# Bioconductor/SparseArray

Hardware: NVIDIA B200
Metric: nnz/s for SVT colSums+colMeans+rowSums+rowVars (na.rm=TRUE), 33538x1e6 int counts d=0.07 per GPU (higher is better)
Workload: dtype int32->f64

## Files before the change

### sparsearray_b200/csrc/svtgpu_colstats.cu

```cuda
#include "svtgpu_internal.h"
#include "svt_ptx.cuh"

#include <stdlib.h>
#include <string.h>

namespace {

enum ColClass { CC_COUNT = 0, CC_SUM, CC_MINMAX, CC_VAR, CC_ANYALL, CC_PROD };

__host__ __device__ inline int col_class_of(int opcode)
{
	switch (opcode) {
	    case SVTGPU_OP_ANYNA: case SVTGPU_OP_COUNTNAS: return CC_COUNT;
	    case SVTGPU_OP_SUM: case SVTGPU_OP_MEAN:       return CC_SUM;
	    case SVTGPU_OP_MIN: case SVTGPU_OP_MAX:        return CC_MINMAX;
	    case SVTGPU_OP_CENTERED_X2_SUM:
	    case SVTGPU_OP_VAR1: case SVTGPU_OP_SD1:       return CC_VAR;
	    case SVTGPU_OP_ANY: case SVTGPU_OP_ALL:        return CC_ANYALL;
	    case SVTGPU_OP_PROD:                           return CC_PROD;
	}
	return -1;
}

struct ColParams {
// ... 330 lines not shown
				}
			}
			for (; i < n; i++) {
				const int x = (int) p[i * 32];
				const bool na = x == SVT_NA_INT;
				const int x0 = na ? 0 : x;
				nna += na;
				s1 += x0;
				s2 += (unsigned int) (x0 * x0);
			}
			SvtColPartial sp;
			svt_col_partial_init(&sp);
			sp.nz = end - start;
			sp.n_na = svt_warp_sum((long long) nna);
			sp.sum = (double) svt_warp_sum((long long) s1);
			unsigned long long t2 = s2;
#pragma unroll
			for (int m = 16; m > 0; m >>= 1)
				t2 += __shfl_xor_sync(SVT_FULL_MASK, t2, m);
			if (lane == 0)
				store_result(P, seg, var_from_int_sums(P.opcode,
						P.narm, P.seg_len, &sp, t2));
			continue;
		}
		LaneAcc<CC, T> acc;
		acc.reset();
		lane_accumulate<CC, T>(acc, vals, start, end, lane);
		SvtColPartial part;
		acc.reduce_into(&part, end - start);
		double center = P.center;
		if (CC == CC_VAR && sizeof(T) == 4 && svt_isnan(center)) {
			int amax = acc.imax;
			unsigned long long s2 = acc.isum2;
#pragma unroll
			for (int m = 16; m > 0; m >>= 1) {
				const int o = __shfl_xor_sync(SVT_FULL_MASK,
							      amax, m);
				amax = o > amax ? o : amax;
				s2 += __shfl_xor_sync(SVT_FULL_MASK, s2, m);
			}
			if (amax < 65536) {
				if (lane == 0)
					store_result(P, seg, var_from_int_sums(
						P.opcode, P.narm, P.seg_len,
						&part, s2));
				continue;
			}
		}
		if (CC == CC_VAR) {
			const bool about_mean = svt_isnan(center);
			if (about_mean)
				center = svt_col_mean(P.is_double, P.narm,
						      P.seg_len, &part);
			bool one_pass = false;
			if (sizeof(T) == 8 && about_mean && P.var_onepass) {
				const double S2 = svt_warp_sum(acc.dsum2);
				const int64_t n_reg = part.nz - part.n_na - part.n_nan;
				const int64_t n = P.seg_len -
					(P.narm ? part.n_na + part.n_nan : 0);
				if (S2 >= 1e-200 && S2 <= 1e200 && n > 0 &&
				    4 * n_reg <= n && !svt_isnan(center)) {
					part.sum2 = S2 - 2.0 * center * part.sum +
						    (double) n_reg * center * center;
					one_pass = true;
				}
			}
			if (!one_pass) {
				double s2 = 0.0;
#pragma unroll 4
				for (int64_t e = start + lane; e < end; e += 32)
					add_sq(s2, vals[e], center);
				part.sum2 = svt_warp_sum(s2);
			}
		}
		if (lane == 0)
			store_result(P, seg, svt_col_finalize(P.opcode,
					P.is_double, P.narm, P.seg_len, center,
					&part));
	}
}

__device__ __forceinline__ void sum_i8_word(uint32_t w, int &s, int &na_bits)
{
	s = __dp4a((int) w, 0x01010101, s);
	na_bits += __popc(__vcmpeq4(w, 0x80808080u));
}

#define SUM_I8_BLOCKS_PER_SM 6
__global__ void __launch_bounds__(256, SUM_I8_BLOCKS_PER_SM)
colstats_sum_i8(ColParams P, const int8_t *__restrict__ v8)
{
	const int lane = threadIdx.x & 31;
	const int64_t warps = ((int64_t) gridDim.x * blockDim.x) >> 5;
	const int64_t gw = ((int64_t) blockIdx.x * blockDim.x + threadIdx.x) >> 5;
	int64_t nstart = 0, nend = 0;
	if (gw < P.nseg) {
		nstart = P.leaf_ptr[gw * P.group];
		nend = P.leaf_ptr[(gw + 1) * P.group];
	}
	for (int64_t seg = gw; seg < P.nseg; seg += warps) {
		const int64_t start = nstart, end = nend;
		if (seg + warps < P.nseg) {
			nstart = P.leaf_ptr[(seg + warps) * P.group];
			nend = P.leaf_ptr[(seg + warps + 1) * P.group];
		}
		long long sum = 0;
		int na_bits = 0;
		const int64_t a16 = (start + 15) & ~(int64_t) 15;
		const int64_t b16 = end & ~(int64_t) 15;
		int64_t lo = start, hi = end;
		if (a16 < b16) {
			const uint4 *q = (const uint4 *) (v8 + a16);
			const int nv = (int) ((b16 - a16) >> 4);
			for (int i = lane; i < nv; i += 128) {
				uint4 u[4];
#pragma unroll
				for (int k = 0; k < 4; k++)
					u[k] = i + 32 * k < nv ? __ldcs(q + i + 32 * k)
							       : make_uint4(0, 0, 0, 0);
				int s = 0;
#pragma unroll
				for (int k = 0; k < 4; k++) {
					sum_i8_word(u[k].x, s, na_bits);
					sum_i8_word(u[k].y, s, na_bits);
					sum_i8_word(u[k].z, s, na_bits);
					sum_i8_word(u[k].w, s, na_bits);
				}
				sum += s;
			}
			if (start + lane < a16) {
				const int x = v8[start + lane];
				sum += x;
				na_bits += x == SVT_COMPACT_NA_I8 ? 8 : 0;
			}
			lo = b16;
		}
		for (int64_t e = lo + lane; e < hi; e += 32) {
			const int x = v8[e];
			sum += x;
			na_bits += x == SVT_COMPACT_NA_I8 ? 8 : 0;
		}
		const long long n_na = svt_warp_sum((long long) na_bits) >> 3;
		sum = svt_warp_sum(sum) + 128 * n_na;
		if (lane == 0) {
			SvtColPartial part;
			svt_col_partial_init(&part);
			part.nz = end - start;
			part.n_na = n_na;
			part.sum = (double) sum;
			store_result(P, seg, svt_col_finalize(P.opcode, P.is_double,
					P.narm, P.seg_len, P.center, &part));
		}
	}
}


#define COL_NS 2

enum {
	IT_FIRST = 1,
	IT_PASS_END = 2,
	IT_PASS2 = 4,
	IT_LAST = 8,
	IT_SINGLE = 16,
	IT_STOP = 32
};

struct __align__(16) ItemMeta {
	int64_t seg;
	int64_t start, end;
	int64_t cbase;
	int32_t celems;
	int32_t flags;
};

template <int CC, typename T>
__device__ __forceinline__ void consume_pass1(LaneAcc<CC, T> &acc,
		const T *buf, int lo, int hi, int lane)
{
	constexpr int VN = Vec16<T>::N;
	const int lo_v = (lo + VN - 1) / VN * VN;
	const int hi_v = hi / VN * VN;
	if (lo_v >= hi_v) {
		for (int e = lo + lane; e < hi; e += 32)
			acc.add(buf[e]);
		return;
	}
	if (lo + lane < lo_v)
		acc.add(buf[lo + lane]);
	if (hi_v + lane < hi)
		acc.add(buf[hi_v + lane]);
	const Vec16<T> *vb = (const Vec16<T> *) buf;
#pragma unroll 2
	for (int v = lo_v / VN + lane; v < hi_v / VN; v += 32) {
		Vec16<T> x = vb[v];
#pragma unroll
		for (int i = 0; i < VN; i++)
			acc.add(x.get(i));
	}
}

template <typename T>
__device__ __forceinline__ void consume_pass2(double &s2, const T *buf,
		int lo, int hi, int lane, double c)
{
	constexpr int VN = Vec16<T>::N;
	const int lo_v = (lo + VN - 1) / VN * VN;
	const int hi_v = hi / VN * VN;
	if (lo_v >= hi_v) {
		for (int e = lo + lane; e < hi; e += 32)
			add_sq(s2, buf[e], c);
		return;
	}
	if (lo + lane < lo_v)
		add_sq(s2, buf[lo + lane], c);
	if (hi_v + lane < hi)
		add_sq(s2, buf[hi_v + lane], c);
	const Vec16<T> *vb = (const Vec16<T> *) buf;
#pragma unroll 2
	for (int v = lo_v / VN + lane; v < hi_v / VN; v += 32) {
		Vec16<T> x = vb[v];
#pragma unroll
		for (int i = 0; i < VN; i++)
			add_sq(s2, x.get(i), c);
	}
}

template <int CC, typename T>
__global__ void __launch_bounds__(512, 1)
colstats_tma(ColParams P, int pairs, int stage_bytes)
{
	extern __shared__ __align__(128) unsigned char smem[];
	unsigned char *data = smem;
	ItemMeta *metas = (ItemMeta *) (smem + (size_t) pairs * COL_NS *
							 stage_bytes);
	uint64_t *bars = (uint64_t *) (metas + pairs * COL_NS);

	const int warp = threadIdx.x >> 5;
	const int lane = threadIdx.x & 31;
	const int pair = warp >> 1;
	const bool is_producer = (warp & 1) == 0;

	if (threadIdx.x == 0) {
		for (int i = 0; i < 2 * pairs * COL_NS; i++)
			svt_mbar_init(svt_smem_u32(&bars[i]), 1);
		svt_mbar_init_fence();
	}
	__syncthreads();

	unsigned char *ring = data + (size_t) pair * COL_NS * stage_bytes;
	ItemMeta *meta = metas + pair * COL_NS;
	const uint32_t full0 = svt_smem_u32(&bars[pair * COL_NS]);
	const uint32_t empty0 = svt_smem_u32(&bars[(pairs + pair) * COL_NS]);
	const int64_t npairs_total = (int64_t) gridDim.x * pairs;
	const int64_t gp = (int64_t) blockIdx.x * pairs + pair;
	constexpr int SZ = (int) sizeof(T);

	if (is_producer) {
		if (lane != 0)
			return;
		const char *vals = (const char *) P.vals;
		const uint64_t policy = svt_policy_evict_first();
		uint32_t it = 0;
		int64_t seg = gp;
		int64_t nstart = 0, nend = 0;
		if (seg < P.nseg) {
			nstart = P.leaf_ptr[seg * P.group];
			nend = P.leaf_ptr[(seg + 1) * P.group];
		}
		while (seg < P.nseg) {
			const int64_t start = nstart, end = nend;
			const int64_t next = seg + npairs_total;
			if (next < P.nseg) {
				nstart = P.leaf_ptr[next * P.group];
				nend = P.leaf_ptr[(next + 1) * P.group];
			}
			const int64_t a0 = (start * SZ) & ~(int64_t) 15;
			const int64_t a1 = (end * SZ + 15) & ~(int64_t) 15;
			const int64_t nch = start == end ? 0
				: (a1 - a0 + stage_bytes - 1) / stage_bytes;
			const int npass = (CC == CC_VAR && nch > 1) ? 2 : 1;
			const int64_t nitems = nch == 0 ? 1 : nch * npass;
			int64_t k = 0;
			for (int pass = 0; pass < npass; pass++) {
			    for (int64_t ch = 0; ch < (nch == 0 ? 1 : nch);
				 ch++, k++) {
				const int st = it % COL_NS;
				svt_mbar_wait(empty0 + 8 * st,
					      ((it / COL_NS) & 1) ^ 1);
				const int64_t ca = a0 + ch * stage_bytes;
				int64_t cb = ca + stage_bytes;
				if (cb > a1) cb = a1;
				const uint32_t bytes = nch == 0 ? 0
						: (uint32_t) (cb - ca);
				ItemMeta md;
				md.seg = seg;
				md.start = start;
				md.end = end;
				md.cbase = ca / SZ;
				md.celems = (int32_t) (bytes / SZ);
				md.flags = (k == 0 ? IT_FIRST : 0) |
					(ch + 1 >= nch ? IT_PASS_END : 0) |
					(pass == 1 ? IT_PASS2 : 0) |
					(k + 1 == nitems ? IT_LAST : 0) |
					(nch <= 1 ? IT_SINGLE : 0);
				meta[st] = md;
// ... 58 lines not shown
				}
			}
		} else {
			consume_pass2<T>(s2, buf, lo, hi, lane, center);
		}
		if (md.flags & IT_LAST) {
			if (CC == CC_VAR)
				part.sum2 = svt_warp_sum(s2);
			if (lane == 0)
				store_result(P, md.seg, svt_col_finalize(
					P.opcode, P.is_double, P.narm,
					P.seg_len, center, &part));
		}
		__syncwarp();
		if (lane == 0)
			svt_mbar_arrive(empty0 + 8 * st);
	}
}

__global__ void __launch_bounds__(256)
colstats_lacunar(ColParams P)
{
	const int64_t stride = (int64_t) gridDim.x * blockDim.x;
	for (int64_t seg = (int64_t) blockIdx.x * blockDim.x + threadIdx.x;
	     seg < P.nseg; seg += stride) {
		const int64_t nz = P.leaf_ptr[(seg + 1) * P.group] -
				   P.leaf_ptr[seg * P.group];
		SvtColPartial part;
		svt_col_partial_ones(&part, nz, 0.0);
		double center = P.center;
		if (svt_col_op_needs_center(P.opcode)) {
			if (svt_isnan(center))
				center = svt_col_mean(P.is_double, P.narm,
						      P.seg_len, &part);
			svt_col_partial_ones(&part, nz, center);
		}
		store_result(P, seg, svt_col_finalize(P.opcode, P.is_double,
				P.narm, P.seg_len, center, &part));
	}
}

template <typename T>
int launch_typed(const ColParams &P, int cc, bool use_tma, int avg_seg_bytes,
		 cudaStream_t stream)
{
	const int sms = svtgpu_sm_count();
	if (!use_tma) {
		int64_t blocks = (P.nseg + 7) / 8;
		if (blocks > (int64_t) sms * 8) blocks = (int64_t) sms * 8;
		if (blocks < 1) blocks = 1;
#define DIRECT(CC) colstats_direct<CC, T><<<(unsigned) blocks, 256, 0, stream>>>(P)
		switch (cc) {
		    case CC_COUNT:  DIRECT(CC_COUNT); break;
		    case CC_SUM:    DIRECT(CC_SUM); break;
		    case CC_MINMAX: DIRECT(CC_MINMAX); break;
		    case CC_VAR:    DIRECT(CC_VAR); break;
		    case CC_ANYALL: DIRECT(CC_ANYALL); break;
		    case CC_PROD:   DIRECT(CC_PROD); break;
		}
#undef DIRECT
		SVT_CUDA(cudaGetLastError());
		svtgpu_count_launch(1);
		return SVTGPU_OK;
	}
	int stage_bytes = (avg_seg_bytes + avg_seg_bytes / 4 + 64 + 1023) /
			  1024 * 1024;
	const int stage_env = atoi(svtgpu_env("SVTGPU_COL_STAGE_KB", "0"));
	if (stage_env > 0) stage_bytes = stage_env * 1024;
	if (stage_bytes < 4096) stage_bytes = 4096;
	if (stage_bytes > 48 * 1024) stage_bytes = 48 * 1024;
	int pairs = (200 * 1024) / (COL_NS * stage_bytes);
	if (pairs > 8) pairs = 8;
	if (pairs < 1) pairs = 1;
	const int pairs_env = atoi(svtgpu_env("SVTGPU_COL_PAIRS", "0"));
	if (pairs_env > 0 && pairs_env <= 8) pairs = pairs_env;
	const size_t smem = (size_t) pairs * COL_NS * stage_bytes +
			    (size_t) pairs * COL_NS * sizeof(ItemMeta) +
			    (size_t) 2 * pairs * COL_NS * sizeof(uint64_t);
	int64_t blocks = (P.nseg + pairs - 1) / pairs;
	if (blocks > sms) blocks = sms;
	if (blocks < 1) blocks = 1;
#define TMA(CC) do { \
		SVT_CUDA(cudaFuncSetAttribute(colstats_tma<CC, T>, \
			cudaFuncAttributeMaxDynamicSharedMemorySize, (int) smem)); \
		colstats_tma<CC, T><<<(unsigned) blocks, pairs * 64, smem, stream>>>( \
			P, pairs, stage_bytes); \
	} while (0)
	switch (cc) {
	    case CC_COUNT:  TMA(CC_COUNT); break;
	    case CC_SUM:    TMA(CC_SUM); break;
	    case CC_MINMAX: TMA(CC_MINMAX); break;
	    case CC_VAR:    TMA(CC_VAR); break;
	    case CC_ANYALL: TMA(CC_ANYALL); break;
	    case CC_PROD:   TMA(CC_PROD); break;
	}
#undef TMA
	SVT_CUDA(cudaGetLastError());
	svtgpu_count_launch(1);
	return SVTGPU_OK;
}

}

int svtgpu_launch_colstats(svtgpu_matrix *m, int opcode, int narm,
			   double center, int64_t group, void *d_out,
			   int32_t *d_warn, cudaStream_t stream)
{
	SVT_ARG(svt_col_op_supported(opcode, m->val_type),
		"colStats: operation %d is not supported on type %d by the "
		"GPU path", opcode, m->val_type);
	SVT_ARG(group >= 1 && (m->nleaf % group) == 0,
		"colStats: 'group' must divide the number of leaves");
	ColParams P;
	P.vals = m->d_vals;
	P.leaf_ptr = m->d_leaf_ptr;
	P.nseg = m->nleaf / group;
	P.group = group;
	P.seg_len = m->nrow * group;
	P.opcode = opcode;
	P.narm = narm != 0;
	P.is_double = svt_is_double(m->val_type);
	P.center = center;
	P.out = d_out;
	P.warn = d_warn;
	P.var_small = 0;
	P.var_onepass = strcmp(svtgpu_env("SVTGPU_COLVAR_DOUBLE", "auto"),
			       "twopass") != 0;
	if (!P.is_double && svt_isnan(center)) {
		const int64_t B = svtgpu_value_bound(m);
		const int64_t per_lane = P.seg_len / 32 + 2;
		if (B >= 0 && B < 46340 &&
		    per_lane < (int64_t) 0x7FFFFFFF / (B * B + 1)) {
			P.var_small = 1;
			if (m->vmax_abs >= 0 && m->vmin >= 0 &&
			    strcmp(svtgpu_env("SVTGPU_COLVAR_NONNEG", "on"),
				   "on") == 0)
				P.var_small = 2;
		}
	}
	if (P.nseg == 0)
		return SVTGPU_OK;
	if (!(m->flags & SVTGPU_HAS_VALS)) {
		int64_t blocks = (P.nseg + 255) / 256;
		int64_t cap = (int64_t) svtgpu_sm_count() * 8;
		if (blocks > cap) blocks = cap;
		colstats_lacunar<<<(unsigned) blocks, 256, 0, stream>>>(P);
		SVT_CUDA(cudaGetLastError());
		svtgpu_count_launch(1);
		return SVTGPU_OK;
	}
	const int cc = col_class_of(opcode);
	if (cc == CC_SUM && !P.is_double) {
		SVT_CHECK(svt_ensure_compact(m, stream));
		if (m->d_vals8 != NULL) {
			int64_t blocks = (P.nseg + 7) / 8;
			const int64_t cap = (int64_t) svtgpu_sm_count() *
					    SUM_I8_BLOCKS_PER_SM;
			if (blocks > cap)
				blocks = cap;
			colstats_sum_i8<<<(unsigned) blocks, 256, 0, stream>>>(
				P, m->d_vals8);
			SVT_CUDA(cudaGetLastError());
			svtgpu_count_launch(1);
			return SVTGPU_OK;
		}
	}
	const char *impl = svtgpu_env("SVTGPU_COLSTATS_IMPL", "direct");
	bool use_tma = strcmp(impl, "tma") == 0 &&
		       (((uintptr_t) m->d_vals) & 15) == 0;
	int64_t avg = m->nnz / P.nseg * (int64_t) svt_val_size(m->val_type);
	if (avg > (1 << 30)) avg = 1 << 30;
	if (P.is_double)
		return launch_typed<double>(P, cc, use_tma, (int) avg, stream);
	return launch_typed<int32_t>(P, cc, use_tma, (int) avg, stream);
}

extern "C" int svtgpu_colstats_out_is_int(int opcode, int val_type)
{
	return svt_col_out_is_int(opcode, val_type);
}

extern "C" int svtgpu_colstats_dev(svtgpu_matrix *m, int opcode, int narm,
				   double center, int64_t group, void *d_out,
				   int32_t *d_warn, void *stream)
{
	SVT_CHECK(svtgpu_require_device());
	SVT_ARG(m != NULL && d_out != NULL, "svtgpu_colstats_dev: NULL argument");
	return svtgpu_launch_colstats(m, opcode, narm, center, group, d_out,
				      d_warn, (cudaStream_t) stream);
}

extern "C" int svtgpu_colstats(svtgpu_matrix *m, int opcode, int narm,
			       double center, int64_t group, void *out,
			       int *warn)
{
	SVT_CHECK(svtgpu_require_device());
	SVT_ARG(m != NULL && out != NULL, "svtgpu_colstats: NULL argument");
	SVT_ARG(group >= 1 && (m->nleaf % group) == 0,
		"colStats: 'group' must divide the number of leaves");
	const int64_t nseg = m->nleaf / group;
	const size_t esz = svt_col_out_is_int(opcode, m->val_type) ? 4 : 8;
	if (warn != NULL)
		*warn = 0;
	m->tm.kernel_ms = m->tm.d2h_ms = 0.0;
	m->tm.d2h_bytes = 0.0;
	m->tm.launches = 0;
	if (nseg == 0)
		return SVTGPU_OK;
	void *scratch = NULL;
	SVT_CHECK(svtgpu_scratch(m, esz * (size_t) nseg + 16, &scratch));
	int32_t *d_warn = (int32_t *) scratch;
	void *d_out = (char *) scratch + 16;
	cudaStream_t s = 0;
	SVT_CUDA(cudaMemsetAsync(d_warn, 0, 16, s));
	SvtTimer t;
	SVT_CHECK(svt_timer_begin(&t, s));
	int64_t l0 = svtgpu_launch_count();
	int rc = svtgpu_launch_colstats(m, opcode, narm, center, group, d_out,
					d_warn, s);
	int rc2 = svt_timer_end(&t, &m->tm.kernel_ms);
	if (rc != SVTGPU_OK)
		return rc;
	SVT_CHECK(rc2);
	m->tm.launches = (int) (svtgpu_launch_count() - l0);
	SVT_CHECK(svt_timer_begin(&t, s));
	int32_t h_warn = 0;
	SVT_CUDA(cudaMemcpyAsync(out, d_out, esz * (size_t) nseg,
				 cudaMemcpyDeviceToHost, s));
	SVT_CUDA(cudaMemcpyAsync(&h_warn, d_warn, sizeof(int32_t),
				 cudaMemcpyDeviceToHost, s));
	SVT_CHECK(svt_timer_end(&t, &m->tm.d2h_ms));
	m->tm.d2h_bytes = (double) (esz * (size_t) nseg);
	if (warn != NULL)
		*warn = h_warn != 0;
	return SVTGPU_OK;
}

namespace {

template <int CC, typename T>
__global__ void __launch_bounds__(256)
summarize_slices(const T *__restrict__ vals, int64_t nnz, int64_t slice,
		 double center, int pass2, SvtColPartial *__restrict__ parts)
{
	const int lane = threadIdx.x & 31;
	const int64_t gw = ((int64_t) blockIdx.x * blockDim.x + threadIdx.x) >> 5;
	const int64_t start = gw * slice;
	if (start >= nnz)
		return;
	const int64_t end = start + slice < nnz ? start + slice : nnz;
	SvtColPartial part;
	if (pass2) {
		double s2 = 0.0;
#pragma unroll 4
		for (int64_t e = start + lane; e < end; e += 32)
			add_sq(s2, vals[e], center);
		svt_col_partial_init(&part);
		part.sum2 = svt_warp_sum(s2);
	} else {
		LaneAcc<CC, T> acc;
		acc.reset();
		lane_accumulate<CC, T>(acc, vals, start, end, lane);
		acc.reduce_into(&part, end - start);
	}
	if (lane == 0)
		parts[gw] = part;
}

__device__ __forceinline__ void col_partial_merge(SvtColPartial *a,
						  const SvtColPartial *b)
{
	a->nz += b->nz;
	a->n_na += b->n_na;
	a->n_nan += b->n_nan;
	a->n_zero += b->n_zero;
	a->sum += b->sum;
	a->sum2 += b->sum2;
	a->prod *= b->prod;
	a->vmin = b->vmin < a->vmin ? b->vmin : a->vmin;
	a->vmax = b->vmax > a->vmax ? b->vmax : a->vmax;
}

__device__ __forceinline__ void col_partial_warp_merge(SvtColPartial *acc)
{
	acc->nz = svt_warp_sum((long long) acc->nz);
	acc->n_na = svt_warp_sum((long long) acc->n_na);
	acc->n_nan = svt_warp_sum((long long) acc->n_nan);
	acc->n_zero = svt_warp_sum((long long) acc->n_zero);
	acc->sum = svt_warp_sum(acc->sum);
	acc->sum2 = svt_warp_sum(acc->sum2);
	acc->prod = svt_warp_prod(acc->prod);
	acc->vmin = svt_warp_min(acc->vmin);
	acc->vmax = svt_warp_max(acc->vmax);
}

__global__ void __launch_bounds__(1024)
summarize_combine(const SvtColPartial *__restrict__ parts, int64_t n,
		  SvtColPartial *__restrict__ out)
{
	__shared__ SvtColPartial warp_part[32];
	const int lane = threadIdx.x & 31;
	const int warp = threadIdx.x >> 5;
	SvtColPartial acc;
	svt_col_partial_init(&acc);
	for (int64_t i = threadIdx.x; i < n; i += blockDim.x) {
		const SvtColPartial p = parts[i];
// ... 301 lines not shown
```

### sparsearray_b200/csrc/svtgpu_internal.h

```cpp
#ifndef SVTGPU_INTERNAL_H
#define SVTGPU_INTERNAL_H

#include <cuda_runtime.h>
#include <stdint.h>
#include <stdio.h>

#include "../../include/svtgpu.h"
#include "svt_semantics.h"

#define SVTGPU_NSTAGE 3
#define SVTGPU_NSPLIT 4

struct svtgpu_matrix {
	int64_t nrow, nleaf, nnz;
	int val_type;
	int flags;
	int owns;
	int device;

	int64_t *d_leaf_ptr;
	int32_t *d_offs;
	void *d_vals;

	cudaStream_t up_stream;
	int64_t stage_cap;
	int32_t *h_offs_stage[SVTGPU_NSTAGE];
	void *h_vals_stage[SVTGPU_NSTAGE];
	cudaEvent_t stage_done[SVTGPU_NSTAGE];
	int stage_busy[SVTGPU_NSTAGE];
	int stage_cur;
	cudaEvent_t up_begin, up_end;
	int up_begun;
	void *d_narrow[SVTGPU_NSTAGE];
	size_t narrow_bytes;

	void *d_scratch;
	size_t scratch_bytes;
	int32_t *d_split[SVTGPU_NSPLIT];
	int split_tile_rows[SVTGPU_NSPLIT];
	int split_ntiles[SVTGPU_NSPLIT];
	int split_next;
	int64_t *d_hist_tiles;
	int64_t hist_tile, hist_ntiles;
	int hist_max_leaves;
	int64_t vmax_abs;
	int64_t n_i8_commits, n_wide_commits;
	int64_t vmin;
	int64_t leaf_base;
	struct svtgpu_matrix *transposed;
	int transpose_failed;
	uint16_t *d_offs16;
	int8_t *d_vals8;
	int compact_state;
	int compact_uses;

	svtgpu_timings tm;
};

#define SVT_COMPACT_NA_I8 (-128)
#define SVT_COMPACT_PAD 64
#define SVT_COMPACT_NONE 0
#define SVT_COMPACT_BUILT 1
#define SVT_COMPACT_INELIGIBLE 2
#define SVT_COMPACT_MAX_ABS 127
#define SVT_COMPACT_MAX_NROW 65536

int svt_ensure_compact(svtgpu_matrix *m, cudaStream_t s);
void svt_drop_compact(svtgpu_matrix *m, cudaStream_t s);

int64_t svtgpu_value_bound(const svtgpu_matrix *m);

void svtgpu_set_error(const char *fmt, ...);
int svtgpu_cuda_fail(cudaError_t e, const char *what, const char *file,
		     int line);

#define SVT_CUDA(call) \
	do { \
		cudaError_t e__ = (call); \
		if (e__ != cudaSuccess) \
			return svtgpu_cuda_fail(e__, #call, __FILE__, __LINE__); \
	} while (0)

#define SVT_CHECK(call) \
	do { \
		int rc__ = (call); \
		if (rc__ != SVTGPU_OK) \
			return rc__; \
	} while (0)

#define SVT_ARG(cond, ...) \
	do { \
		if (!(cond)) { \
			svtgpu_set_error(__VA_ARGS__); \
			return SVTGPU_ERR_ARG; \
		} \
	} while (0)

cudaError_t svt_malloc_async(void **out, size_t bytes, cudaStream_t s);
cudaError_t svt_free_async(void *p, cudaStream_t s);

int svtgpu_require_device(void);
void svtgpu_count_launch(int n);
int svtgpu_scratch(svtgpu_matrix *m, size_t bytes, void **ptr);
int svtgpu_sm_count(void);
const char *svtgpu_env(const char *name, const char *dflt);

static inline int svt_is_double(int val_type)
{
	return val_type == SVTGPU_DOUBLE;
}

static inline size_t svt_val_size(int val_type)
{
	return val_type == SVTGPU_DOUBLE ? sizeof(double) : sizeof(int32_t);
}

int svtgpu_ensure_absmax(svtgpu_matrix *m, cudaStream_t s);
int svtgpu_ensure_split(svtgpu_matrix *m, int nstrips, int strip_rows,
			cudaStream_t s, const int32_t **split);
int svtgpu_ensure_transpose(svtgpu_matrix *m, cudaStream_t s,
			    svtgpu_matrix **out);
int svtgpu_launch_colstats(svtgpu_matrix *m, int opcode, int narm,
			   double center, int64_t group, void *d_out,
			   int32_t *d_warn, cudaStream_t stream);
int svtgpu_launch_row_accumulate(svtgpu_matrix *m, int opcode, int narm,
				 int want_sum2, double *d_state,
				 cudaStream_t stream);
int svtgpu_launch_row_finalize(int opcode, int val_type, int narm,
			       int64_t nrow, int64_t nstrata,
			       const double *d_center, const double *d_state,
			       void *d_out, int32_t *d_warn,
			       cudaStream_t stream);
int svtgpu_launch_row_moments_finalize(int val_type, int narm, int64_t nrow,
				       int64_t nstrata, const double *d_state,
				       double *d_mean, double *d_var,
				       cudaStream_t stream);

struct SvtTimer {
	cudaEvent_t a, b;
	cudaStream_t s;
	int ok;
};
int svt_timer_begin(SvtTimer *t, cudaStream_t s);
int svt_timer_end(SvtTimer *t, double *ms);

#endif
```

### sparsearray_b200/csrc/svtgpu_rowstats.cu

```cuda
#include "svtgpu_internal.h"
#include "svt_ptx.cuh"

#include <string.h>

namespace {

enum RowClass { RC_COUNT = 0, RC_SUM, RC_X2, RC_MINMAX };

inline int row_class_of(int opcode)
{
	switch (opcode) {
	    case SVTGPU_OP_ANYNA: case SVTGPU_OP_COUNTNAS: return RC_COUNT;
	    case SVTGPU_OP_SUM:                            return RC_SUM;
	    case SVTGPU_OP_CENTERED_X2_SUM:                return RC_X2;
	    case SVTGPU_OP_MIN: case SVTGPU_OP_MAX:        return RC_MINMAX;
	}
	return -1;
}

__device__ __forceinline__ int classify(int32_t x, double &v)
{
	v = (double) x;
	return x == SVT_NA_INT ? 1 : 0;
}
// ... 1425 lines not shown
	     base += (int64_t) HIST_THREADS * U) {
		int o[U], x[U];
#pragma unroll
		for (int k = 0; k < U; k++) {
			const int64_t e = base +
				(int64_t) k * HIST_THREADS;
			const bool ok = e < end;
			o[k] = ok ? P.offs[e] : -1;
			x[k] = (ok && !LACUNAR) ? P.vals[e] : 1;
		}
#pragma unroll
		for (int k = 0; k < U; k++) {
			if (o[k] < 0)
				continue;
			if (MODE == HIST_COUNT16) {
				atomicAdd(&cell[o[k] >> 1],
					  1u << ((o[k] & 1) * 16));
			} else if (x[k] == SVT_NA_INT) {
				atomicAdd(&P.state[SVT_ROW_SLOT_NA *
					P.nrow + o[k]], 1.0);
			} else if (MODE == HIST_MOMENTS) {
				const unsigned int v =
					(unsigned int) x[k];
				atomicAdd(&cell[o[k]],
					  v * ((v << 16) + 1u));
			} else if (MODE == HIST_MAX32) {
				atomicMax(&cell[o[k]],
					  (unsigned int) x[k] + 1u);
			} else {
				atomicAdd(&cell[o[k]],
					  (unsigned int) x[k]);
			}
		}
	}
	};
	auto add8 = [&](const uint32_t o, const int x) {
		if (x == SVT_COMPACT_NA_I8) {
			atomicAdd(&P.state[SVT_ROW_SLOT_NA * P.nrow + o], 1.0);
		} else if (MODE == HIST_MOMENTS) {
			const unsigned int v = (unsigned int) x;
			hist_red(cell_s + (o << 2), v * ((v << 16) + 1u));
		} else {
			hist_red(cell_s + (o << 2), (unsigned int) x);
		}
	};
	auto stream8 = [&](const int64_t start, const int64_t end) {
	constexpr int K = 2;
	int64_t head = (8 - (start & 7)) & 7;
	if (head > end - start)
		head = end - start;
	if ((int64_t) threadIdx.x < head)
		add8(P.offs16[start + threadIdx.x], P.vals8[start + threadIdx.x]);
	const int64_t vstart = start + head;
	const int64_t nfull = (end - vstart) / ((int64_t) HIST_THREADS * 8 * K);
	const int4 *po = (const int4 *) (P.offs16 + vstart) + threadIdx.x;
	const uint2 *pv = (const uint2 *) (P.vals8 + vstart) + threadIdx.x;
	int4 o_nx[K];
	uint2 v_nx[K];
	auto request = [&]() {
#pragma unroll
		for (int k = 0; k < K; k++) {
			o_nx[k] = ldg_stream_v4(po + k * HIST_THREADS);
			v_nx[k] = ldg_stream_v2(pv + k * HIST_THREADS);
		}
		po += K * HIST_THREADS;
		pv += K * HIST_THREADS;
	};
	if (nfull > 0)
		request();
	for (int64_t b = 0; b < nfull; b++) {
		int4 o[K];
		uint2 v[K];
#pragma unroll
		for (int k = 0; k < K; k++) {
			o[k] = o_nx[k];
			v[k] = v_nx[k];
		}
		if (b + 1 < nfull)
			request();
#pragma unroll
		for (int k = 0; k < K; k++) {
			const uint32_t ow[4] = { (uint32_t) o[k].x, (uint32_t) o[k].y,
						 (uint32_t) o[k].z, (uint32_t) o[k].w };
			const uint32_t vw[2] = { v[k].x, v[k].y };
#pragma unroll
			for (int j = 0; j < 8; j++)
				add8((ow[j >> 1] >> ((j & 1) * 16)) & 0xFFFFu,
				     (int) (int8_t) (vw[j >> 2] >> ((j & 3) * 8)));
		}
	}
	for (int64_t e = vstart + nfull * HIST_THREADS * 8 * K + threadIdx.x;
	     e < end; e += HIST_THREADS)
		add8(P.offs16[e], P.vals8[e]);
	};
	auto feed = [&](const int64_t start, const int64_t end) {
		if (NARROW)
			stream8(start, end);
		else
			stream(start, end);
	};
	auto checkpoint = [&](const bool last) {
	__syncthreads();
	if (MODE == HIST_MOMENTS && !last) {
		int risky = 0;
		for (int64_t r = threadIdx.x; r < P.nrow;
		     r += blockDim.x)
			risky |= (cell[r] & 0x80008000u) != 0;
		if (!__syncthreads_or(risky))
			return;
	}
	for (int64_t r = threadIdx.x; r < P.nrow;
	     r += blockDim.x) {
		if (MODE == HIST_MAX32) {
			const unsigned int c = cell[r];
			if (c != 0) {
				atomic_max_double(&P.state[
					SVT_ROW_SLOT_EXT * P.nrow + r],
					(double) (c - 1u));
				atomicAdd(&P.state[SVT_ROW_SLOT_CVG *
					P.nrow + r], 1.0);
			}
			continue;
		}
		if (MODE == HIST_MOMENTS) {
			const unsigned int c = cell[r];
			if (c != 0) {
				atomicAdd(&P.state[SVT_ROW_SLOT_SUM *
					P.nrow + r],
					(double) (c & 0xFFFFu));
				atomicAdd(&P.state[SVT_ROW_SLOT_SUM2 *
					P.nrow + r],
					(double) (c >> 16));
			}
			continue;
		}
		const int v = LACUNAR
			? (int) ((cell[r >> 1] >> ((r & 1) * 16))
				 & 0xFFFFu)
			: (int) cell[r];
		if (v != 0)
			atomicAdd(&P.state[SVT_ROW_SLOT_SUM *
				P.nrow + r], (double) v);
	}
	__syncthreads();
	if (!last) {
		for (int64_t i = threadIdx.x; i < ncell;
		     i += blockDim.x)
			cell[i] = 0;
		__syncthreads();
	}

	};

	if (P.tile_leaf != NULL) {
		for (int64_t i = threadIdx.x; i < ncell; i += blockDim.x)
			cell[i] = 0;
		__syncthreads();
		int64_t used = 0;
		int64_t t = blockIdx.x;
		int64_t la = 0, lb = 0;
		if (t < P.ntiles) {
			la = P.tile_leaf[t];
			lb = P.tile_leaf[t + 1];
		}
		while (t < P.ntiles) {
			const int64_t L = lb - la + 1;
			const int64_t tn = t + gridDim.x;
			int64_t na = 0, nb = 0;
			if (tn < P.ntiles) {
				na = P.tile_leaf[tn];
				nb = P.tile_leaf[tn + 1];
			}
			if (used + L > P.piece_leaves) {
				checkpoint(false);
				used = 0;
			}
			used += L;
			const int64_t start = t * P.tile;
			feed(start, start + P.tile < P.nnz ? start + P.tile
							   : P.nnz);
			t = tn;
			la = na;
			lb = nb;
		}
		checkpoint(true);
		return;
	}

	for (int chunk_i = blockIdx.x; chunk_i < P.nchunks; chunk_i += gridDim.x) {
		int chunk = chunk_i;
		if (P.back_first && P.nchunks == 2 * (int) gridDim.x)
			chunk = chunk_i < (int) gridDim.x ? chunk_i + (int) gridDim.x
							  : chunk_i - (int) gridDim.x;
		int64_t bounds[2];
		for (int k = 0; k < 2; k++) {
			const int c = chunk + k;
			if (c >= P.nchunks) { bounds[k] = P.nleaf; continue; }
			const int64_t target = (int64_t) ((double) P.nnz *
					((double) c / (double) P.nchunks));
			int64_t lo = 0, hi = P.nleaf;
			while (lo < hi) {
				const int64_t mid = lo + ((hi - lo) >> 1);
				if (P.leaf_ptr[mid] < target) lo = mid + 1;
				else                          hi = mid;
			}
			bounds[k] = c == 0 ? 0 : lo;
		}
		for (int64_t i = threadIdx.x; i < ncell; i += blockDim.x)
			cell[i] = 0;
		__syncthreads();
		for (int64_t p0 = bounds[0]; p0 < bounds[1];
		     p0 += P.piece_leaves) {
			const int64_t p1 = p0 + P.piece_leaves < bounds[1]
					   ? p0 + P.piece_leaves : bounds[1];
			feed(P.leaf_ptr[p0], P.leaf_ptr[p1]);
			checkpoint(p1 == bounds[1]);
		}
	}
}

__global__ void __launch_bounds__(256)
hist_tile_leaves(const int64_t *__restrict__ leaf_ptr, int64_t nleaf,
		 int64_t nnz, int64_t tile, int64_t ntiles,
		 int64_t *__restrict__ tile_leaf, int *max_leaves, int pass)
{
	const int64_t t = (int64_t) blockIdx.x * blockDim.x + threadIdx.x;
	if (t > ntiles)
		return;
	if (pass == 0) {
		int64_t e = t * tile;
		if (e > nnz - 1) e = nnz - 1;
		int64_t lo = 0, hi = nleaf;
		while (lo < hi) {
			const int64_t mid = lo + ((hi - lo) >> 1);
			if (leaf_ptr[mid + 1] <= e) lo = mid + 1;
			else                        hi = mid;
		}
		tile_leaf[t] = lo;
	} else if (t < ntiles) {
		const int64_t L = tile_leaf[t + 1] - tile_leaf[t] + 1;
		atomicMax(max_leaves, L > INT32_MAX ? INT32_MAX : (int) L);
	}
}

int launch_row_hist(svtgpu_matrix *m, int mode, int64_t max_abs,
		    double *d_state, cudaStream_t s)
{
	const bool lac = mode == HIST_COUNT16;
	RowHistParams P;
	memset(&P, 0, sizeof(P));
	P.offs = m->d_offs;
	P.vals = lac ? NULL : (const int32_t *) m->d_vals;
	P.leaf_ptr = m->d_leaf_ptr;
	P.nleaf = m->nleaf;
	P.nnz = m->nnz;
	P.nrow = m->nrow;
	bool narrow = false;
	if (mode == HIST_SUM32 || mode == HIST_MOMENTS) {
		SVT_CHECK(svt_ensure_compact(m, s));
		narrow = m->d_offs16 != NULL && m->d_vals8 != NULL;
		P.offs16 = m->d_offs16;
		P.vals8 = m->d_vals8;
	}
	const int sms = svtgpu_sm_count();
	P.nchunks = (int64_t) sms * 2 < m->nleaf ? sms * 2
						 : (m->nleaf > 0 ? (int) m->nleaf : 1);
	const int64_t M = max_abs > 0 ? max_abs : 1;
	const int64_t lim = mode == HIST_COUNT16 ? 65535
			  : mode == HIST_MAX32 ? ((int64_t) 1 << 30)
			  : mode == HIST_MOMENTS ? 32767 / (M * M)
			  : (int64_t) INT32_MAX / M;
	P.piece_leaves = (int) (lim < 1 ? 1 : lim > (1 << 30) ? (1 << 30) : lim);
	const int forced = atoi(svtgpu_env("SVTGPU_ROW_HIST_PIECE", "0"));
	if (forced > 0 && forced < P.piece_leaves)
		P.piece_leaves = forced;
	P.state = d_state;
	P.back_first = strcmp(svtgpu_env("SVTGPU_ROW_HIST_ORDER", "back"),
			      "back") == 0;
	P.lacunar_vec = atoi(svtgpu_env("SVTGPU_ROW_HIST_LACUNAR_VEC", "1")) &&
			(((uintptr_t) m->d_offs) & 15) == 0;
	const size_t smem = lac ? 4 * (size_t) ((m->nrow + 1) / 2)
				: 4 * (size_t) m->nrow;
	int grid = P.nchunks < sms ? P.nchunks : sms;
	const int64_t tile = (int64_t) HIST_THREADS * (lac ? 16 : 8) * 4;
	const int64_t ntiles = (m->nnz + tile - 1) / tile;
	if (ntiles >= (int64_t) sms * 4 &&
	    strcmp(svtgpu_env("SVTGPU_ROW_HIST_TILES", "cyclic"), "cyclic") == 0) {
		if (m->d_hist_tiles == NULL || m->hist_tile != tile) {
			if (m->d_hist_tiles != NULL)
				svt_free_async(m->d_hist_tiles, s);
			m->d_hist_tiles = NULL;
			int *d_max = NULL;
			SVT_CUDA(svt_malloc_async((void **) &m->d_hist_tiles,
					8 * (size_t) (ntiles + 1) + 64, s));
			d_max = (int *) (m->d_hist_tiles + ntiles + 1);
			SVT_CUDA(cudaMemsetAsync(d_max, 0, sizeof(int), s));
			const unsigned g = (unsigned) ((ntiles + 1 + 255) / 256);
			hist_tile_leaves<<<g, 256, 0, s>>>(m->d_leaf_ptr, m->nleaf,
				m->nnz, tile, ntiles, m->d_hist_tiles, d_max, 0);
			hist_tile_leaves<<<g, 256, 0, s>>>(m->d_leaf_ptr, m->nleaf,
				m->nnz, tile, ntiles, m->d_hist_tiles, d_max, 1);
			SVT_CUDA(cudaGetLastError());
			svtgpu_count_launch(2);
			int h_max = 0;
			SVT_CUDA(cudaMemcpyAsync(&h_max, d_max, sizeof(int),
					cudaMemcpyDeviceToHost, s));
			SVT_CUDA(cudaStreamSynchronize(s));
			m->hist_tile = tile;
			m->hist_ntiles = ntiles;
			m->hist_max_leaves = h_max;
		}
		if (m->hist_max_leaves <= P.piece_leaves) {
			P.tile_leaf = m->d_hist_tiles;
			P.tile = tile;
			P.ntiles = ntiles;
			grid = sms;
		}
	}
#define HIST_LAUNCH(MODE, NARROW) do { \
		SVT_CUDA(cudaFuncSetAttribute(row_hist<MODE, NARROW>, \
			cudaFuncAttributeMaxDynamicSharedMemorySize, (int) smem)); \
		row_hist<MODE, NARROW><<<grid, HIST_THREADS, smem, s>>>(P); \
	} while (0)
	if (mode == HIST_COUNT16)      HIST_LAUNCH(HIST_COUNT16, false);
	else if (mode == HIST_MOMENTS && narrow) HIST_LAUNCH(HIST_MOMENTS, true);
	else if (mode == HIST_MOMENTS) HIST_LAUNCH(HIST_MOMENTS, false);
	else if (mode == HIST_MAX32)   HIST_LAUNCH(HIST_MAX32, false);
	else if (narrow)               HIST_LAUNCH(HIST_SUM32, true);
	else                           HIST_LAUNCH(HIST_SUM32, false);
#undef HIST_LAUNCH
	SVT_CUDA(cudaGetLastError());
	svtgpu_count_launch(1);
	return SVTGPU_OK;
}

__global__ void __launch_bounds__(256)
row_lacunar_derive(double *state, int64_t nrow, int want_sum2)
{
	const int64_t r = (int64_t) blockIdx.x * blockDim.x + threadIdx.x;
	if (r >= nrow)
		return;
	const double n = state[SVT_ROW_SLOT_SUM * nrow + r];
	if (want_sum2)
		state[SVT_ROW_SLOT_SUM2 * nrow + r] = n;
	else if (n > 0.0)
		state[SVT_ROW_SLOT_EXT * nrow + r] = 1.0;
}

__global__ void __launch_bounds__(256)
row_max_hist_coverage(double *state, int64_t nrow)
{
	const int64_t r = (int64_t) blockIdx.x * blockDim.x + threadIdx.x;
	if (r < nrow)
		state[SVT_ROW_SLOT_CVG * nrow + r] +=
			state[SVT_ROW_SLOT_NA * nrow + r];
}

int ensure_absmax(svtgpu_matrix *m, cudaStream_t s)
{
	if (m->vmax_abs >= 0)
		return SVTGPU_OK;
	if (!(m->flags & SVTGPU_HAS_VALS) || m->nnz == 0) {
		m->vmax_abs = 1;
		m->vmin = 0;
		return SVTGPU_OK;
	}
	unsigned long long *d_max = NULL, h_max[2] = { 0, 0 };
	SVT_CUDA(svt_malloc_async((void **) &d_max, 2 * sizeof(*d_max), s));
	cudaError_t e = cudaMemsetAsync(d_max, 0, 2 * sizeof(*d_max), s);
	if (e == cudaSuccess) {
		absmax_int<<<grid_for(m->nnz, 256 * 16), 256, 0, s>>>(
			(const int32_t *) m->d_vals, m->nnz, d_max);
		e = cudaGetLastError();
		svtgpu_count_launch(1);
	}
	if (e == cudaSuccess)
		e = cudaMemcpyAsync(h_max, d_max, sizeof(h_max),
				    cudaMemcpyDeviceToHost, s);
	if (e == cudaSuccess)
		e = cudaStreamSynchronize(s);
	svt_free_async(d_max, s);
	SVT_CUDA(e);
	m->vmax_abs = (int64_t) h_max[0];
	m->vmin = h_max[1] > 0 ? -1 : 0;
	return SVTGPU_OK;
}

template <int RC, typename T, bool LAC>
int launch_flat(const svtgpu_matrix *m, int is_min, double *d_state,
		cudaStream_t s)
{
	row_flat<RC, T, LAC><<<grid_for(m->nnz, 256 * 8), 256, 0, s>>>(
		m->d_offs, (const T *) m->d_vals, m->nnz, m->nrow, is_min,
		d_state);
	SVT_CUDA(cudaGetLastError());
	svtgpu_count_launch(1);
	return SVTGPU_OK;
}

template <int RC, typename T, bool LAC, typename ACC>
int launch_tiles(svtgpu_matrix *m, const TileConfig &c, int is_min,
		 int64_t flush_leaves, double *d_state, cudaStream_t s)
{
	constexpr int NACC = RC == RC_SUM ? 1 : 2;
	const int32_t *split = NULL;
	SVT_CHECK(ensure_split(m, c, s, &split));
	void *part = NULL;
	SVT_CHECK(svtgpu_scratch(m, sizeof(double) * (size_t) c.nchunks *
				 NACC * (size_t) m->nrow + 64, &part));
	RowTileParams P;
	P.offs = m->d_offs;
	P.vals = LAC ? NULL : m->d_vals;
	P.leaf_ptr = m->d_leaf_ptr;
	P.split = split;
	P.nleaf = m->nleaf;
	P.nnz = m->nnz;
	P.nrow = m->nrow;
	P.ntiles = c.ntiles;
	P.tile_rows = c.tile_rows;
	P.nchunks = c.nchunks;
	P.stage_elems = c.stage_elems;
	P.is_min = is_min;
	P.flush_leaves = flush_leaves;
	P.part = (double *) part;
	P.state = d_state;
	SVT_CUDA(cudaFuncSetAttribute(row_tiles<RC, T, LAC, ACC>,
		cudaFuncAttributeMaxDynamicSharedMemorySize, (int) c.smem));
	row_tiles<RC, T, LAC, ACC><<<(unsigned) (c.nchunks * c.ntiles),
				     ROW_THREADS, c.smem, s>>>(P);
	SVT_CUDA(cudaGetLastError());
	row_combine<RC><<<grid_for(m->nrow, 256), 256, 0, s>>>(
		(const double *) part, c.nchunks, m->nrow, is_min, d_state);
	SVT_CUDA(cudaGetLastError());
	svtgpu_count_launch(2);
	return SVTGPU_OK;
}

struct StripConfig {
	int ok;
	int ntiles, nchunks, nstrips, strip_rows, warps;
	int slots;
	size_t smem;
};

StripConfig choose_strips(int64_t nrow, int64_t nleaf, int64_t nnz, int nacc,
			  int acc_size)
{
	StripConfig c;
	memset(&c, 0, sizeof(c));
	const int sms = svtgpu_sm_count();
	const size_t budget = (size_t) 227 * 1024 - 1024 - 256;
	const double avg_leaf = nleaf > 0 ? (double) nnz / (double) nleaf : 0.0;
	int force_w = atoi(svtgpu_env("SVTGPU_ROW_WARPS", "0"));
	int force_t = atoi(svtgpu_env("SVTGPU_ROW_NTILES", "0"));
	for (int nt = force_t > 0 ? force_t : 1; nt <= 64; nt++) {
		int W = force_w;
		if (W <= 0) {
			double per_tile = avg_leaf / nt;
			W = (int) (per_tile / 60.0 + 0.5);
			if (W < 4) W = 4;
			if (W > 16) W = 16;
			if (nacc == 2 && acc_size == 8 && per_tile >= 16 * 24.0)
				W = 16;
		}
// ... 577 lines not shown
```

Baseline: 1991 billion.

## Add tile-balanced int8 column-sum kernel and software-pipelined narrow row histogram

Adds a nnz-tiled column-sum path for compact int8 values. Each block sums fixed 32K-entry tiles with dp4a and packed NA counting, accumulates per-segment in shared memory, and a second kernel stitches segments that span tiles using head/tail partials. The narrow row-histogram path gains a register double-buffered streaming loop over whole tiles, and tile-table construction is factored into a shared helper so both row and column stats can reuse one table of the same tile size. The intent is to fix load imbalance from variable column lengths and hide load latency. The cost is an extra launch, a temporary allocation per call, and a host sync when the table is built.

```diff
diff --git a/sparsearray_b200/csrc/svtgpu_colstats.cu b/sparsearray_b200/csrc/svtgpu_colstats.cu
--- a/sparsearray_b200/csrc/svtgpu_colstats.cu
+++ b/sparsearray_b200/csrc/svtgpu_colstats.cu
@@ -506,6 +506,244 @@
 					P.narm, P.seg_len, P.center, &part));
 		}
 	}
+}
+
+#define SUMT_THREADS 512
+#define SUMT_V (SVT_TILE_ENTRIES / 16 / SUMT_THREADS)
+#define SUMT_MAX_SEG 256
+
+struct SumTileArgs {
+	const int8_t *v8;
+	const int64_t *tile_leaf;
+	int64_t ntiles, nnz;
+	long long *head, *tail;
+};
+
+__device__ __forceinline__ void sum_na_word(uint32_t w, int &s, int &na)
+{
+	s = __dp4a((int) w, 0x01010101, s);
+	const uint32_t t = (w & 0x7F7F7F7Fu) + 0x7F7F7F7Fu;
+	na += __popc(~t & w & 0x80808080u);
+}
+
+__device__ __forceinline__ uint32_t chunk_mask(int a, int b, int j)
+{
+	const int lo = a - 4 * j > 0 ? a - 4 * j : 0;
+	const int hi = b - 4 * j < 4 ? b - 4 * j : 4;
+	if (hi <= lo)
+		return 0u;
+	const uint32_t top = hi == 4 ? 0xFFFFFFFFu : (1u << (8 * hi)) - 1u;
+	return top & ~((1u << (8 * lo)) - 1u);
+}
+
+__device__ __forceinline__ int chunk_packed(const uint4 &u, int a, int b)
+{
+	int s = 0, na = 0;
+	const uint32_t w[4] = { u.x, u.y, u.z, u.w };
+#pragma unroll
+	for (int j = 0; j < 4; j++)
+		sum_na_word(w[j] & chunk_mask(a, b, j), s, na);
+	return s + 128 * na + (na << 18);
+}
+
+__device__ __forceinline__ void unpack_warp(int r, int &sum, int &na)
+{
+	na = (r + (1 << 17)) >> 18;
+	sum = r - (na << 18);
+}
+
+__device__ __forceinline__ unsigned long long acc_word(long long sum,
+						       long long na)
+{
+	return (unsigned long long) ((na << 32) + sum);
+}
+
+__device__ __forceinline__ void acc_split(unsigned long long a, long long &sum,
+					  long long &na)
+{
+	sum = (long long) (int) (uint32_t) a;
+	na = (long long) ((a - (unsigned long long) sum) >> 32);
+}
+
+__device__ __forceinline__ void finalize_sum(const ColParams &P, int64_t seg,
+					     int64_t nz, long long sum,
+					     long long na)
+{
+	SvtColPartial part;
+	svt_col_partial_init(&part);
+	part.nz = nz;
+	part.n_na = na;
+	part.sum = (double) sum;
+	store_result(P, seg, svt_col_finalize(P.opcode, P.is_double, P.narm,
+					      P.seg_len, P.center, &part));
+}
+
+__global__ void __launch_bounds__(SUMT_THREADS, 2)
+colsum_i8_tiles(ColParams P, SumTileArgs A)
+{
+	__shared__ int bnd[SUMT_MAX_SEG + 1];
+	__shared__ int64_t gbnd[SUMT_MAX_SEG + 1];
+	__shared__ unsigned long long acc[SUMT_MAX_SEG];
+	const int lane = threadIdx.x & 31;
+	const int warp = threadIdx.x >> 5;
+	const int64_t tile = SVT_TILE_ENTRIES;
+
+	uint4 nx[SUMT_V];
+	int64_t nbound = 0;
+	auto request = [&](const int64_t tt, const int64_t a, const int64_t b) {
+		const int64_t t0 = tt * tile;
+		const int64_t len = A.nnz - t0 < tile ? A.nnz - t0 : tile;
+		const uint4 *q = (const uint4 *) (A.v8 + t0);
+#pragma unroll
+		for (int k = 0; k < SUMT_V; k++) {
+			const int c = k * SUMT_THREADS + (int) threadIdx.x;
+			nx[k] = 16 * (int64_t) c < len ? __ldcs(q + c)
+						       : make_uint4(0, 0, 0, 0);
+		}
+		const int64_t k0 = a / P.group, S = b / P.group - k0 + 1;
+		if ((int64_t) threadIdx.x <= S)
+			nbound = P.leaf_ptr[(k0 + threadIdx.x) * P.group];
+	};
+
+	int64_t t = blockIdx.x;
+	int64_t la = 0, lb = 0, la1 = 0, lb1 = 0;
+	if (t < A.ntiles) {
+		la = A.tile_leaf[t];
+		lb = A.tile_leaf[t + 1];
+		request(t, la, lb);
+		if (t + gridDim.x < A.ntiles) {
+			la1 = A.tile_leaf[t + gridDim.x];
+			lb1 = A.tile_leaf[t + gridDim.x + 1];
+		}
+	}
+	for (; t < A.ntiles; t += gridDim.x) {
+		uint4 cur[SUMT_V];
+#pragma unroll
+		for (int k = 0; k < SUMT_V; k++)
+			cur[k] = nx[k];
+		const int64_t bound = nbound;
+		const int64_t k0 = la / P.group;
+		const int S = (int) (lb / P.group - k0 + 1);
+		const int64_t t0 = t * tile;
+		const int len = (int) (A.nnz - t0 < tile ? A.nnz - t0 : tile);
+		const int64_t tn = t + gridDim.x;
+		if (tn < A.ntiles) {
+			request(tn, la1, lb1);
+			la = la1;
+			lb = lb1;
+			if (tn + gridDim.x < A.ntiles) {
+				la1 = A.tile_leaf[tn + gridDim.x];
+				lb1 = A.tile_leaf[tn + gridDim.x + 1];
+			}
+		}
+		if ((int) threadIdx.x <= S) {
+			gbnd[threadIdx.x] = bound;
+			const int64_t r = bound - t0;
+			bnd[threadIdx.x] = r < 0 ? 0 : r > len ? len : (int) r;
+		}
+		if ((int) threadIdx.x < S)
+			acc[threadIdx.x] = 0ull;
+		__syncthreads();
+		auto seg_of = [&](const int x) {
+			int lo = 0, hi = S - 1;
+			while (lo < hi) {
+				const int mid = (lo + hi + 1) >> 1;
+				if (bnd[mid] <= x) lo = mid;
+				else               hi = mid - 1;
+			}
+			return lo;
+		};
+#pragma unroll
+		for (int k = 0; k < SUMT_V; k++) {
+			const int p0 = (k * SUMT_THREADS + warp * 32) * 16;
+			if (p0 >= len)
+				continue;
+			const int span = len - p0 < 512 ? len - p0 : 512;
+			const int p = p0 + lane * 16;
+			const int i0 = seg_of(p0);
+			const int e0 = bnd[i0 + 1];
+			if (e0 >= p0 + span) {
+				const int r = __reduce_add_sync(SVT_FULL_MASK,
+						chunk_packed(cur[k], 0, 16));
+				if (lane == 0) {
+					int s, na;
+					unpack_warp(r, s, na);
+					atomicAdd(&acc[i0], acc_word(s, na));
+				}
+				continue;
+			}
+			const int i1 = seg_of(p0 + span - 1);
+			const int s1 = bnd[i1];
+			const int rf = __reduce_add_sync(SVT_FULL_MASK,
+					chunk_packed(cur[k], 0, e0 - p));
+			const int rl = __reduce_add_sync(SVT_FULL_MASK,
+					chunk_packed(cur[k], s1 - p, 16));
+			if (lane == 0) {
+				int s, na;
+				unpack_warp(rf, s, na);
+				atomicAdd(&acc[i0], acc_word(s, na));
+				unpack_warp(rl, s, na);
+				atomicAdd(&acc[i1], acc_word(s, na));
+			}
+			int x = e0 > p ? e0 : p;
+			const int xe = s1 < p + 16 ? s1 : p + 16;
+			while (x < xe) {
+				const int i = seg_of(x);
+				const int e = bnd[i + 1] < xe ? bnd[i + 1] : xe;
+				int s, na;
+				unpack_warp(chunk_packed(cur[k], x - p, e - p), s, na);
+				atomicAdd(&acc[i], acc_word(s, na));
+				x = e;
+			}
+		}
+		__syncthreads();
+		if ((int) threadIdx.x < S) {
+			const int i = threadIdx.x;
+			long long sum, na;
+			acc_split(acc[i], sum, na);
+			const int64_t s = gbnd[i], e = gbnd[i + 1];
+			if (s >= t0 && e <= t0 + len) {
+				finalize_sum(P, k0 + i, e - s, sum, na);
+			} else {
+				if (i == 0)
+					A.head[t] = (long long) acc[i];
+				if (i == S - 1)
+					A.tail[t] = (long long) acc[i];
+			}
+		}
+		__syncthreads();
+	}
+}
+
+__global__ void __launch_bounds__(256)
+colsum_i8_edges(ColParams P, SumTileArgs A)
+{
+	const int64_t x = (int64_t) blockIdx.x * blockDim.x + threadIdx.x;
+	const int64_t nth = (int64_t) gridDim.x * blockDim.x;
+	const int64_t tile = SVT_TILE_ENTRIES;
+	if (x < A.ntiles) {
+		const int64_t t0 = x * tile;
+		const int64_t t1 = A.nnz - t0 < tile ? A.nnz : t0 + tile;
+		const int64_t k = A.tile_leaf[x + 1] / P.group;
+		const int64_t s = P.leaf_ptr[k * P.group];
+		const int64_t e = P.leaf_ptr[(k + 1) * P.group];
+		if (s >= t0 && s < t1 && e > t1) {
+			long long sum, na, ps, pn;
+			acc_split((unsigned long long) A.tail[x], sum, na);
+			for (int64_t v = x + 1; v * tile < e; v++) {
+				acc_split((unsigned long long) A.head[v], ps, pn);
+				sum += ps;
+				na += pn;
+			}
+			finalize_sum(P, k, e - s, sum, na);
+		}
+	}
+	const int64_t lead = A.tile_leaf[0] / P.group;
+	for (int64_t k = x; k < lead; k += nth)
+		finalize_sum(P, k, 0, 0, 0);
+	for (int64_t k = A.tile_leaf[A.ntiles] / P.group + 1 + x; k < P.nseg;
+	     k += nth)
+		finalize_sum(P, k, 0, 0, 0);
 }
 
 
@@ -870,6 +1108,35 @@
 	const int cc = col_class_of(opcode);
 	if (cc == CC_SUM && !P.is_double) {
 		SVT_CHECK(svt_ensure_compact(m, stream));
+		const int64_t ntiles = (m->nnz + SVT_TILE_ENTRIES - 1) /
+				       SVT_TILE_ENTRIES;
+		const int sms = svtgpu_sm_count();
+		if (m->d_vals8 != NULL && ntiles >= sms &&
+		    (((uintptr_t) m->d_vals8) & 15) == 0) {
+			SVT_CHECK(svt_ensure_tile_table(m, SVT_TILE_ENTRIES,
+							stream));
+			if (m->hist_max_leaves <= SUMT_MAX_SEG) {
+				SumTileArgs A;
+				A.v8 = m->d_vals8;
+				A.tile_leaf = m->d_hist_tiles;
+				A.ntiles = ntiles;
+				A.nnz = m->nnz;
+				SVT_CUDA(svt_malloc_async((void **) &A.head,
+					2 * sizeof(long long) * (size_t) ntiles,
+					stream));
+				A.tail = A.head + ntiles;
+				const int64_t grid = ntiles < 2 * (int64_t) sms
+						     ? ntiles : 2 * (int64_t) sms;
+				colsum_i8_tiles<<<(unsigned) grid, SUMT_THREADS, 0,
+						  stream>>>(P, A);
+				colsum_i8_edges<<<(unsigned) ((ntiles + 255) / 256),
+						  256, 0, stream>>>(P, A);
+				SVT_CUDA(cudaGetLastError());
+				SVT_CUDA(svt_free_async(A.head, stream));
+				svtgpu_count_launch(2);
+				return SVTGPU_OK;
+			}
+		}
 		if (m->d_vals8 != NULL) {
 			int64_t blocks = (P.nseg + 7) / 8;
 			const int64_t cap = (int64_t) svtgpu_sm_count() *
diff --git a/sparsearray_b200/csrc/svtgpu_internal.h b/sparsearray_b200/csrc/svtgpu_internal.h
--- a/sparsearray_b200/csrc/svtgpu_internal.h
+++ b/sparsearray_b200/csrc/svtgpu_internal.h
@@ -67,6 +67,9 @@
 
 int svt_ensure_compact(svtgpu_matrix *m, cudaStream_t s);
 void svt_drop_compact(svtgpu_matrix *m, cudaStream_t s);
+
+#define SVT_TILE_ENTRIES 32768
+int svt_ensure_tile_table(svtgpu_matrix *m, int64_t tile, cudaStream_t s);
 
 int64_t svtgpu_value_bound(const svtgpu_matrix *m);
 
diff --git a/sparsearray_b200/csrc/svtgpu_rowstats.cu b/sparsearray_b200/csrc/svtgpu_rowstats.cu
--- a/sparsearray_b200/csrc/svtgpu_rowstats.cu
+++ b/sparsearray_b200/csrc/svtgpu_rowstats.cu
@@ -1601,6 +1601,80 @@
 
 	};
 
+	if (NARROW && P.tile_leaf != NULL) {
+		constexpr int K = 2;
+		constexpr int64_t BATCH = (int64_t) HIST_THREADS * 8 * K;
+		const int NB = (int) (P.tile / BATCH);
+		const int64_t nwhole = P.nnz / P.tile;
+		for (int64_t i = threadIdx.x; i < ncell; i += blockDim.x)
+			cell[i] = 0;
+		__syncthreads();
+		int4 o_nx[K];
+		uint2 v_nx[K];
+		auto request = [&](const int64_t first) {
+			const int4 *po = (const int4 *) (P.offs16 + first) + threadIdx.x;
+			const uint2 *pv = (const uint2 *) (P.vals8 + first) + threadIdx.x;
+#pragma unroll
+			for (int k = 0; k < K; k++) {
+				o_nx[k] = ldg_stream_v4(po + k * HIST_THREADS);
+				v_nx[k] = ldg_stream_v2(pv + k * HIST_THREADS);
+			}
+		};
+		int64_t used = 0;
+		int64_t t = blockIdx.x;
+		int64_t la = 0, lb = 0;
+		if (t < P.ntiles) {
+			la = P.tile_leaf[t];
+			lb = P.tile_leaf[t + 1];
+		}
+		if (t < nwhole)
+			request(t * P.tile);
+		for (; t < nwhole; t += gridDim.x) {
+			const int64_t L = lb - la + 1;
+			const int64_t tn = t + gridDim.x;
+			if (tn < P.ntiles) {
+				la = P.tile_leaf[tn];
+				lb = P.tile_leaf[tn + 1];
+			}
+			for (int j = 0; j < NB; j++) {
+				int4 o[K];
+				uint2 v[K];
+#pragma unroll
+				for (int k = 0; k < K; k++) {
+					o[k] = o_nx[k];
+					v[k] = v_nx[k];
+				}
+				if (j + 1 < NB)
+					request(t * P.tile + (j + 1) * BATCH);
+				else if (tn < nwhole)
+					request(tn * P.tile);
+				if (j == 0) {
+					if (used + L > P.piece_leaves) {
+						checkpoint(false);
+						used = 0;
+					}
+					used += L;
+				}
+#pragma unroll
+				for (int k = 0; k < K; k++) {
+					const uint32_t ow[4] = { (uint32_t) o[k].x, (uint32_t) o[k].y,
+								 (uint32_t) o[k].z, (uint32_t) o[k].w };
+					const uint32_t vw[2] = { v[k].x, v[k].y };
+#pragma unroll
+					for (int i = 0; i < 8; i++)
+						add8((ow[i >> 1] >> ((i & 1) * 16)) & 0xFFFFu,
+						     (int) (int8_t) (vw[i >> 2] >> ((i & 3) * 8)));
+				}
+			}
+		}
+		if (t < P.ntiles) {
+			if (used + (lb - la + 1) > P.piece_leaves)
+				checkpoint(false);
+			stream8(t * P.tile, P.nnz);
+		}
+		checkpoint(true);
+		return;
+	}
 	if (P.tile_leaf != NULL) {
 		for (int64_t i = threadIdx.x; i < ncell; i += blockDim.x)
 			cell[i] = 0;
@@ -1691,6 +1765,40 @@
 		atomicMax(max_leaves, L > INT32_MAX ? INT32_MAX : (int) L);
 	}
 }
+
+}
+
+int svt_ensure_tile_table(svtgpu_matrix *m, int64_t tile, cudaStream_t s)
+{
+	if (m->d_hist_tiles != NULL && m->hist_tile == tile)
+		return SVTGPU_OK;
+	const int64_t ntiles = (m->nnz + tile - 1) / tile;
+	if (m->d_hist_tiles != NULL)
+		svt_free_async(m->d_hist_tiles, s);
+	m->d_hist_tiles = NULL;
+	m->hist_tile = 0;
+	SVT_CUDA(svt_malloc_async((void **) &m->d_hist_tiles,
+				  8 * (size_t) (ntiles + 1) + 64, s));
+	int *d_max = (int *) (m->d_hist_tiles + ntiles + 1);
+	SVT_CUDA(cudaMemsetAsync(d_max, 0, sizeof(int), s));
+	const unsigned g = (unsigned) ((ntiles + 1 + 255) / 256);
+	hist_tile_leaves<<<g, 256, 0, s>>>(m->d_leaf_ptr, m->nleaf, m->nnz,
+		tile, ntiles, m->d_hist_tiles, d_max, 0);
+	hist_tile_leaves<<<g, 256, 0, s>>>(m->d_leaf_ptr, m->nleaf, m->nnz,
+		tile, ntiles, m->d_hist_tiles, d_max, 1);
+	SVT_CUDA(cudaGetLastError());
+	svtgpu_count_launch(2);
+	int h_max = 0;
+	SVT_CUDA(cudaMemcpyAsync(&h_max, d_max, sizeof(int),
+				 cudaMemcpyDeviceToHost, s));
+	SVT_CUDA(cudaStreamSynchronize(s));
+	m->hist_tile = tile;
+	m->hist_ntiles = ntiles;
+	m->hist_max_leaves = h_max;
+	return SVTGPU_OK;
+}
+
+namespace {
 
 int launch_row_hist(svtgpu_matrix *m, int mode, int64_t max_abs,
 		    double *d_state, cudaStream_t s)
@@ -1731,34 +1839,11 @@
 	const size_t smem = lac ? 4 * (size_t) ((m->nrow + 1) / 2)
 				: 4 * (size_t) m->nrow;
 	int grid = P.nchunks < sms ? P.nchunks : sms;
-	const int64_t tile = (int64_t) HIST_THREADS * (lac ? 16 : 8) * 4;
+	const int64_t tile = lac ? 2 * SVT_TILE_ENTRIES : SVT_TILE_ENTRIES;
 	const int64_t ntiles = (m->nnz + tile - 1) / tile;
 	if (ntiles >= (int64_t) sms * 4 &&
 	    strcmp(svtgpu_env("SVTGPU_ROW_HIST_TILES", "cyclic"), "cyclic") == 0) {
-		if (m->d_hist_tiles == NULL || m->hist_tile != tile) {
-			if (m->d_hist_tiles != NULL)
-				svt_free_async(m->d_hist_tiles, s);
-			m->d_hist_tiles = NULL;
-			int *d_max = NULL;
-			SVT_CUDA(svt_malloc_async((void **) &m->d_hist_tiles,
-					8 * (size_t) (ntiles + 1) + 64, s));
-			d_max = (int *) (m->d_hist_tiles + ntiles + 1);
-			SVT_CUDA(cudaMemsetAsync(d_max, 0, sizeof(int), s));
-			const unsigned g = (unsigned) ((ntiles + 1 + 255) / 256);
-			hist_tile_leaves<<<g, 256, 0, s>>>(m->d_leaf_ptr, m->nleaf,
-				m->nnz, tile, ntiles, m->d_hist_tiles, d_max, 0);
-			hist_tile_leaves<<<g, 256, 0, s>>>(m->d_leaf_ptr, m->nleaf,
-				m->nnz, tile, ntiles, m->d_hist_tiles, d_max, 1);
-			SVT_CUDA(cudaGetLastError());
-			svtgpu_count_launch(2);
-			int h_max = 0;
-			SVT_CUDA(cudaMemcpyAsync(&h_max, d_max, sizeof(int),
-					cudaMemcpyDeviceToHost, s));
-			SVT_CUDA(cudaStreamSynchronize(s));
-			m->hist_tile = tile;
-			m->hist_ntiles = ntiles;
-			m->hist_max_leaves = h_max;
-		}
+		SVT_CHECK(svt_ensure_tile_table(m, tile, s));
 		if (m->hist_max_leaves <= P.piece_leaves) {
 			P.tile_leaf = m->d_hist_tiles;
 			P.tile = tile;
```

New measurement: 1699 billion (median of 6 runs). 0.854x the previous value.
